# microsoft/fadtk

Measured on NVIDIA H100. Metric: audio_seconds_embedded_per_second, higher is better.
Workload: dtype f16

## Files before the change

fadtk_b200/_native.py:

```python
from __future__ import annotations

import ctypes as C
import os
from pathlib import Path

import numpy as np
import torch

_LIB_PATH = Path(os.environ.get("FADTK_B200_LIB") or Path(__file__).parent / "csrc" / "libfadtk_b200.so")
_lib = None

c_ll = C.c_longlong
c_vp = C.c_void_p


class NativeError(RuntimeError):
    pass


class VggishWeights(C.Structure):
    _fields_ = [("conv1_w_host", c_vp), ("conv1_b_host", c_vp),
                ("conv_w_host", c_vp * 5), ("conv_b_host", c_vp * 5),
                ("fc_w_host", c_vp * 3), ("fc_b_host", c_vp * 3), ("split_mask", C.c_uint32)]


SIGNATURES = {
    "fad_version": (C.c_int, []),
    "fad_last_error": (C.c_char_p, []),
    "fad_create": (C.c_int, [C.c_int, C.c_int, C.POINTER(c_vp)]),
    "fad_destroy": (C.c_int, [c_vp]),
    "fad_vggish_load": (C.c_int, [c_vp, C.POINTER(VggishWeights)]),
    "fad_vggish_num_examples": (c_ll, [c_ll]),
    "fad_vggish_plan": (c_ll, [c_vp, c_ll, c_vp, c_ll, c_vp]),
    "fad_vggish_forward": (C.c_int, [c_vp, c_vp, c_vp, c_ll, c_vp, c_vp]),
    "fad_vggish_logmel": (C.c_int, [c_vp, c_vp, c_vp, c_ll, c_vp, C.c_int, c_vp]),
    "fad_vggish_conv1": (C.c_int, [c_vp, c_vp, c_ll, c_vp, c_vp]),
    "fad_umma_layer": (C.c_int, [c_vp, c_vp, C.c_int, C.c_int, C.c_int, C.c_int, c_vp, c_vp,
                                 C.c_int, C.c_int, C.c_int, C.c_int, C.c_int, c_vp, c_vp, c_vp]),
    "fad_linear": (C.c_int, [c_vp, c_vp, c_ll, C.c_int, c_ll, c_vp, C.c_int, c_vp, C.c_int, C.c_int, c_vp, c_vp,
                             c_vp, C.c_int, C.c_int, C.c_int, c_vp]),
    "fad_clap_load": (C.c_int, [c_vp, c_vp, C.c_int, C.c_int]),
    "fad_clap_plan": (c_ll, [c_vp, c_ll, c_vp, c_vp, c_ll, c_vp]),
    "fad_clap_plan_frames": (c_ll, [c_vp, c_ll, c_vp, c_vp, c_vp, c_ll, c_vp]),
    "fad_clap_forward": (C.c_int, [c_vp, c_vp, c_vp, c_vp, c_vp, c_ll, c_vp, c_ll, c_vp, c_vp]),
    "fad_clap_logmel": (C.c_int, [c_vp, c_vp, c_vp, c_vp, c_vp, c_ll, c_vp, c_vp]),
    "fad_clap_patch_embed": (C.c_int, [c_vp, c_vp, c_ll, c_vp, c_ll, c_vp, c_vp]),
    "fad_clap_block": (C.c_int, [c_vp, C.c_int, c_vp, c_ll, c_vp, c_vp]),
    "fad_clap_merge": (C.c_int, [c_vp, C.c_int, c_vp, c_ll, c_vp, c_vp]),
    "fad_clap_head": (C.c_int, [c_vp, c_vp, c_ll, c_vp, c_vp]),
    "fad_stats_acc_len": (C.c_size_t, [C.c_int]),
    "fad_stats_accumulate": (C.c_int, [c_vp, c_vp, c_ll, C.c_int, c_vp, c_vp, C.c_int, c_vp]),
    "fad_stats_accumulate_gather": (C.c_int, [c_vp, c_vp, c_ll, c_vp, c_ll, C.c_int, c_vp, c_vp, c_vp]),
    "fad_stats_finalize": (C.c_int, [c_vp, c_vp, c_vp, C.c_int, c_vp, c_vp, c_vp]),
    "fad_file_means": (C.c_int, [c_vp, c_vp, c_ll, C.c_int, C.c_int, c_vp, c_vp, c_vp]),
    "fad_stats_accumulate_f64": (C.c_int, [c_vp, c_vp, c_ll, C.c_int, c_vp, c_vp]),
    "fad_stats_finalize_mirrored": (C.c_int, [c_vp, c_vp, c_vp, c_vp, c_vp, C.c_int, C.c_int, c_vp, c_vp, c_vp]),
    "fad_frechet": (C.c_int, [c_vp, c_vp, c_vp, c_vp, c_vp, C.c_int, C.c_int, c_vp, c_vp]),
    "fad_sqrt_psd": (C.c_int, [c_vp, c_vp, C.c_int, C.c_int, c_vp, c_vp, c_vp]),
    "fad_frechet_presqrt": (C.c_int, [c_vp, c_vp, c_vp, c_vp, c_vp, c_vp, C.c_int, C.c_int, c_vp, c_vp]),
    "fad_whisper_load": (C.c_int, [c_vp, c_vp, c_vp, C.c_int, C.c_int]),
    "fad_whisper_forward": (C.c_int, [c_vp, c_vp, c_vp, c_vp, c_ll, c_vp, c_vp]),
    "fad_whisper_logmel": (C.c_int, [c_vp, c_vp, c_vp, c_vp, c_ll, c_vp, c_vp]),
    "fad_whisper_conv": (C.c_int, [c_vp, C.c_int, c_vp, c_vp, c_ll, c_vp, c_vp]),
    "fad_whisper_enc_layer": (C.c_int, [c_vp, C.c_int, c_vp, c_ll, c_vp, c_vp]),
    "fad_whisper_encode": (C.c_int, [c_vp, c_vp, c_vp, c_vp, c_ll, c_vp, c_vp]),
    "fad_whisper_dec_layer": (C.c_int, [c_vp, C.c_int, c_vp, c_vp, c_ll, c_vp, c_vp]),
    "fad_w2v_load": (C.c_int, [c_vp, c_vp, c_vp, C.c_int, C.c_int, C.c_int]),
    "fad_w2v_forward": (C.c_int, [c_vp, c_vp, c_ll, C.c_int, C.c_int, c_vp, c_vp]),
    "fad_w2v_normalize": (C.c_int, [c_vp, c_vp, c_ll, C.c_int, c_vp, c_vp]),
    "fad_w2v_conv": (C.c_int, [c_vp, C.c_int, c_vp, c_ll, C.c_int, c_vp, c_vp]),
    "fad_w2v_posconv": (C.c_int, [c_vp, c_vp, c_ll, C.c_int, c_vp, c_vp]),
    "fad_w2v_layer": (C.c_int, [c_vp, C.c_int, c_vp, c_ll, C.c_int, c_vp, c_vp]),
    "fad_encodec_load": (C.c_int, [c_vp, c_vp, C.c_int, c_ll, C.c_int]),
    "fad_encodec_forward": (C.c_int, [c_vp, c_vp, c_ll, C.c_int, c_vp, c_vp]),
    "fad_encodec_conv": (C.c_int, [c_vp, C.c_int, c_vp, c_ll, C.c_int, C.c_int, C.c_int, c_vp, c_vp]),
    "fad_encodec_lstm": (C.c_int, [c_vp, c_vp, c_ll, C.c_int, c_vp, c_vp]),
    "fad_resample_geometry": (C.c_int, [C.c_int, C.c_int, c_vp, c_vp, c_vp, c_vp]),
    "fad_resample_length": (c_ll, [C.c_int, C.c_int, c_ll]),
    "fad_resample_bank": (C.c_int, [C.c_int, C.c_int, c_vp]),
    "fad_resample": (C.c_int, [c_vp, c_vp, c_vp, C.c_int, c_ll, C.c_int, C.c_int, c_vp, c_vp, c_vp]),
    "fad_frechet_batched": (C.c_int, [c_vp, c_vp, c_vp, c_vp, c_vp, c_vp, c_ll, C.c_int, C.c_int, c_vp, c_vp]),
    "fad_attention": (C.c_int, [c_vp, c_vp, c_ll, C.c_int, C.c_int, c_vp, C.c_int, c_vp]),
    "fad_window_attention": (C.c_int, [c_vp, c_vp, c_ll, C.c_int, C.c_int, c_vp, C.c_int, C.c_int, c_vp, c_vp]),
    "fad_attention_bias": (C.c_int, [c_vp, c_vp, c_ll, C.c_int, C.c_int, c_vp, c_vp, c_vp, c_vp]),
    "fad_wavlm_gate": (C.c_int, [c_vp, c_vp, c_vp, c_vp, c_vp, c_ll, C.c_int, C.c_int, c_vp, c_vp]),
    "fad_wavlm_bias_table": (C.c_int, [C.c_int, C.c_int, c_vp, c_vp]),
    "fad_decoder_self_attention": (C.c_int, [c_vp, c_vp, c_ll, C.c_int, c_vp, c_vp]),
    "fad_cross_attention": (C.c_int, [c_vp, c_vp, c_vp, c_ll, C.c_int, C.c_int, c_vp, c_vp]),
    "fad_layernorm": (C.c_int, [c_vp, c_vp, c_vp, c_vp, c_ll, C.c_int, C.c_int, C.c_int, C.c_int, C.c_int, C.c_int,
                                c_vp, c_vp, c_vp]),
    "fad_bench_dmma_peak": (C.c_int, [c_vp, C.c_int, c_vp]),
    "fad_kad_median_sq": (C.c_int, [c_vp, c_vp, c_ll, C.c_int, c_vp, c_vp]),
    "fad_kad_sums": (C.c_int, [c_vp, c_vp, c_ll, c_ll, C.c_int, c_vp, c_vp, c_vp]),
    "fad_kad_song_sums": (C.c_int, [c_vp, c_vp, c_ll, c_vp, c_ll, C.c_int, c_vp, c_vp, c_vp]),
    "fad_kad_median_sq_sharded": (C.c_int, [c_vp, c_vp, C.c_int, c_vp, c_ll, C.c_int, c_vp, c_vp]),
    "fad_kad_sums_sharded": (C.c_int, [c_vp, c_vp, C.c_int, c_vp, c_ll, c_ll, C.c_int, c_vp, c_vp, c_vp]),
    "fad_kad_song_sums_sharded": (C.c_int, [c_vp, c_vp, C.c_int, c_vp, c_ll, c_vp, c_ll, C.c_int, c_vp, c_vp, c_vp]),
    "fad_kad_shard_plan": (C.c_int, [c_vp, c_ll, C.c_int, c_vp]),
    "fad_knn_radii_sq": (C.c_int, [c_vp, c_vp, c_ll, c_ll, C.c_int, C.c_int, c_vp, c_vp]),
    "fad_prdc_counts": (C.c_int, [c_vp, c_vp, c_ll, c_ll, C.c_int, c_vp, c_vp, c_vp, c_vp]),
    "fad_comm_unique_id": (C.c_int, [c_vp]),
    "fad_comm_init": (C.c_int, [c_vp, c_vp, C.c_int, C.c_int]),
    "fad_comm_destroy": (C.c_int, [c_vp]),
    "fad_stats_allreduce": (C.c_int, [c_vp, c_vp, c_vp, C.c_int, c_vp]),
    "fad_allreduce_sum_f64": (C.c_int, [c_vp, c_vp, c_vp, c_ll, c_vp]),
    "fad_launch_count": (c_ll, [c_vp]),
    "fad_profile_enable": (C.c_int, [c_vp, C.c_int]),
    "fad_profile_collect": (C.c_int, [c_vp, c_vp, c_vp, C.c_int]),
}

PROF_CATEGORIES = 20
PROF_NAMES = {0: "logmel", 1: "conv1", 2: "conv2", 3: "conv3_1", 4: "conv3_2", 5: "conv4_1", 6: "conv4_2",
              7: "fc1", 8: "fc2", 9: "fc3", 10: "stats", 11: "stats_reduce", 12: "frechet",
              13: "clap_front", 14: "clap_gemm", 15: "clap_attn", 16: "clap_other"}


def library_path() -> Path:
    return _LIB_PATH


def lib():
    global _lib
    if _lib is None:
        if not _LIB_PATH.exists():
            raise NativeError(
                f"{_LIB_PATH} is missing - run `python -c 'import __graft_entry__ as g; g.build()'`. "
                "fadtk_b200 has no CPU fallback.")
        _lib = C.CDLL(str(_LIB_PATH))
        for name, (res, args) in SIGNATURES.items():
            fn = getattr(_lib, name)
            fn.restype = res
            fn.argtypes = args
    return _lib


def _check(rc: int):
    if rc != 0:
        raise NativeError(lib().fad_last_error().decode())


def _stream() -> int:
    return torch.cuda.current_stream().cuda_stream


def _ptr(t) -> int:
    return 0 if t is None else t.data_ptr()


class Engine:

    def __init__(self, device: int | None = None, max_examples: int = 2048):
        if not torch.cuda.is_available():
            raise NativeError("no CUDA device visible: fadtk_b200 has no CPU fallback")
        self.device = torch.cuda.current_device() if device is None else int(device)
        self.max_examples = int(max_examples)
        h = c_vp()
        _check(lib().fad_create(self.device, self.max_examples, C.byref(h)))
        self._h = h
        self._keep = []
        self.has_comm = False
        self.owners = {}

    def close(self):
        if getattr(self, "_h", None):
            lib().fad_destroy(self._h)
            self._h = None

    def __del__(self):
        try:
            self.close()
        except Exception:
            pass

    @property
    def torch_device(self):
        return torch.device("cuda", self.device)

    @property
    def launches(self) -> int:
        return int(lib().fad_launch_count(self._h))

    @staticmethod
    def comm_unique_id() -> bytes:
        buf = C.create_string_buffer(128)
        _check(lib().fad_comm_unique_id(buf))
        return buf.raw

    def comm_init(self, unique_id: bytes, rank: int, world: int):
        assert len(unique_id) == 128
        _check(lib().fad_comm_init(self._h, C.create_string_buffer(unique_id, 128), int(rank), int(world)))
        self.has_comm = True

    def allreduce_sum_(self, buf: torch.Tensor) -> torch.Tensor:
        assert buf.dtype == torch.float64 and buf.is_cuda and buf.is_contiguous()
        _check(lib().fad_allreduce_sum_f64(self._h, None, buf.data_ptr(), buf.numel(), _stream()))
        return buf

    def attention(self, qkv: torch.Tensor, n_clips: int, legacy: bool = False) -> torch.Tensor:
        assert qkv.dtype == torch.float16 and qkv.is_cuda and qkv.is_contiguous() and qkv.shape[0] % n_clips == 0
        S, d = qkv.shape[0] // n_clips, qkv.shape[1] // 3
        out = torch.empty((qkv.shape[0], d), dtype=torch.float16, device=qkv.device)
        _check(lib().fad_attention(self._h, qkv.data_ptr(), n_clips, S, d, out.data_ptr(), int(legacy), _stream()))
        return out

    def window_attention(self, qkv, n_windows: int, C: int, heads: int, relbias, res: int, shift: int, out):
        _check(lib().fad_window_attention(self._h, _ptr(qkv), int(n_windows), int(C), int(heads), _ptr(relbias),
                                          int(res), int(shift), _ptr(out), _stream()))
        return out

    def attention_bias(self, qkv, n_clips: int, S: int, d: int, relb, gate, out):
        _check(lib().fad_attention_bias(self._h, _ptr(qkv), int(n_clips), int(S), int(d), _ptr(relb), _ptr(gate),
                                        _ptr(out), _stream()))
        return out

    def wavlm_gate(self, x, w, b, c, rows: int, heads: int, d: int, out):
        _check(lib().fad_wavlm_gate(self._h, _ptr(x), _ptr(w), _ptr(b), _ptr(c), int(rows), int(heads), int(d),
                                    _ptr(out), _stream()))
        return out

    @staticmethod
    def wavlm_bias_table(rel_embed: np.ndarray, S: int) -> np.ndarray:
        emb = np.ascontiguousarray(rel_embed, dtype=np.float32)
        out = np.empty((emb.shape[1], max(2 * int(S) - 1, 0)), dtype=np.float32)
        _check(lib().fad_wavlm_bias_table(emb.shape[1], int(S), emb.ctypes.data, out.ctypes.data))
        return out

    def decoder_self_attention(self, qkv, n_clips: int, d: int, out):
        _check(lib().fad_decoder_self_attention(self._h, _ptr(qkv), int(n_clips), int(d), _ptr(out), _stream()))
        return out

    def cross_attention(self, q, kv, n_clips: int, S: int, d: int, out):
        _check(lib().fad_cross_attention(self._h, _ptr(q), _ptr(kv), int(n_clips), int(S), int(d), _ptr(out), _stream()))
        return out

    def layernorm(self, x, gamma, beta, rows: int, C: int, ld_out: int, out16, out32=None, *, res: int = 0,
                  shift: int = 0, mode: int = 0, gelu: bool = False):
        _check(lib().fad_layernorm(self._h, _ptr(x), _ptr(gamma), _ptr(beta), int(rows), int(C), int(ld_out), int(res),
                                   int(shift), int(mode), int(gelu), _ptr(out16), _ptr(out32), _stream()))
        return out16

    def dmma_peak_tflops(self, iters: int = 0) -> float:
        out = C.c_double(0.0)
        _check(lib().fad_bench_dmma_peak(self._h, int(iters), C.byref(out)))
        return float(out.value)

    def profile(self, on: bool):
        _check(lib().fad_profile_enable(self._h, int(on)))

    def profile_collect(self, reset: bool = True) -> dict:
        ms = (C.c_double * PROF_CATEGORIES)()
        cnt = (c_ll * PROF_CATEGORIES)()
        _check(lib().fad_profile_collect(self._h, ms, cnt, int(reset)))
        return {PROF_NAMES[i]: (ms[i], int(cnt[i])) for i in PROF_NAMES if cnt[i]}

    def vggish_load(self, packed: dict):
        self.owners.pop("vggish", None)
        w = VggishWeights()
        keep = {k: v.contiguous() for k, v in packed.items() if hasattr(v, "contiguous")}
        w.conv1_w_host = keep["conv1.w"].data_ptr()
        w.conv1_b_host = keep["conv1.b"].data_ptr()
        for i in range(5):
            w.conv_w_host[i] = keep[f"conv{i + 2}.w"].data_ptr()
            w.conv_b_host[i] = keep[f"conv{i + 2}.b"].data_ptr()
        for i in range(3):
            w.fc_w_host[i] = keep[f"fc{i + 1}.w"].data_ptr()
            w.fc_b_host[i] = keep[f"fc{i + 1}.b"].data_ptr()
        w.split_mask = int(packed.get("split_mask", 0))
        _check(lib().fad_vggish_load(self._h, C.byref(w)))

    @staticmethod
    def vggish_plan(clip_offsets: np.ndarray):
        off = np.ascontiguousarray(clip_offsets, dtype=np.int64)
        n_clips = off.shape[0] - 1
        rows = np.empty(n_clips, dtype=np.int64)
        n = lib().fad_vggish_plan(off.ctypes.data, n_clips, None, 0, rows.ctypes.data)
        ex = np.empty(n, dtype=np.int64)
        lib().fad_vggish_plan(off.ctypes.data, n_clips, ex.ctypes.data, n, None)
        return ex, rows

    def vggish_forward(self, pcm: torch.Tensor, ex_start: torch.Tensor, out: torch.Tensor | None = None):
        assert pcm.dtype == torch.int16 and pcm.is_cuda and pcm.is_contiguous()
        assert ex_start.dtype == torch.int64 and ex_start.is_cuda
        n = ex_start.shape[0]
        if out is None:
            out = torch.empty((n, 128), dtype=torch.float16, device=pcm.device)
# ... 432 lines not shown
```

fadtk_b200/csrc/fadtk_b200.cu:

```cuda
#include "../../include/fadtk_b200.h"

#include <cuda.h>
#include <cuda_runtime.h>
#include <cuda_fp16.h>
#include <cxxabi.h>
#include <algorithm>
#include <cmath>
#include <cstdio>
#include <cstdlib>
#include <cstring>
#include <memory>
#include <set>
#include <string>
#include <type_traits>
#include <utility>
#include <vector>

#include "conv_gemm.cuh"
#include "frontend.cuh"
#include "stats.cuh"
#include "frechet.cuh"
#include "clap.cuh"
#include "resample.cuh"
#include "whisper.cuh"
// ... 429 lines not shown
    if (!h) return fail("null handle");
    h->prof_on = on != 0;
    return 0;
}

int fad_profile_collect(fad_handle* h, double* ms_out, long long* count_out, int reset) {
    if (!h) return fail("null handle");
    CK(cudaSetDevice(h->device));
    CK(cudaDeviceSynchronize());
    for (const auto& sp : h->spans) {
        float ms = 0.f;
        if (cudaEventElapsedTime(&ms, h->ev_pool[sp.e0], h->ev_pool[sp.e1]) == cudaSuccess) {
            h->prof_ms[sp.cat] += ms; h->prof_count[sp.cat]++;
        }
    }
    h->spans.clear(); h->ev_used = 0;
    for (int i = 0; i < FAD_PROF_CATEGORIES; ++i) {
        if (ms_out) ms_out[i] = h->prof_ms[i];
        if (count_out) count_out[i] = h->prof_count[i];
        if (reset) { h->prof_ms[i] = 0.0; h->prof_count[i] = 0; }
    }
    return 0;
}
const char* fad_last_error(void) { return g_err.c_str(); }

int fad_create(int device, int max_examples, fad_handle** out) {
    if (!out) return fail("null out pointer");
    int count = 0;
    if (cudaGetDeviceCount(&count) != cudaSuccess || count == 0)
        return fail("no CUDA device: fadtk_b200 has no CPU fallback");
    if (device < 0 || device >= count) return fail("bad device index");
    CK(cudaSetDevice(device));
    cudaDeviceProp prop;
    CK(cudaGetDeviceProperties(&prop, device));
    if (prop.major != 9) return fail("fadtk_b200 kernels are built for sm_90a (Hopper H100) only");
    std::unique_ptr<fad_handle> h(new fad_handle());
    h->device = device;
    h->num_sms = prop.multiProcessorCount;
    h->max_examples = max_examples > 0 ? max_examples : 2048;

    std::vector<double> tw, hann, melw; std::vector<int> ms, mc;
    build_frontend_tables(tw, hann, melw, ms, mc);
    if (upload(h->mem, &h->d_twiddle, tw.data(), tw.size() * 8) || upload(h->mem, &h->d_hann, hann.data(), hann.size() * 8) ||
        upload(h->mem, &h->d_melw, melw.data(), melw.size() * 8) || upload(h->mem, &h->d_mel_start, ms.data(), ms.size() * 4) ||
        upload(h->mem, &h->d_mel_count, mc.data(), mc.size() * 4)) return 1;
    const auto smem = [](const void* kernel, size_t bytes) {
        return cudaFuncSetAttribute(kernel, cudaFuncAttributeMaxDynamicSharedMemorySize, (int)bytes);
    };
    CK(smem((const void*)fad::logmel_kernel<double>, fad::logmel_smem_bytes<double>()));
    CK(smem((const void*)fad::logmel_kernel<float>, fad::logmel_smem_bytes<float>()));
    CK(smem((const void*)fad::clap_logmel_kernel, fad::clap_logmel_smem_bytes()));
    CK(smem((const void*)fad::attention_wgmma_kernel, fad::kAtSmem));
    CK(smem((const void*)fad::clap_window_attention_kernel<24>, fad::att_smem_bytes(24, fad::kAttWarps, fad::kAttStages)));
    CK(smem((const void*)fad::clap_window_attention_kernel<32>, fad::att_smem_bytes(32, fad::kAttWarps, fad::kAttStages)));
    CK(smem((const void*)fad::kad_tile_kernel<0>, fad::kKadSmemBytes));
    CK(smem((const void*)fad::kad_tile_kernel<1>, fad::kKadSmemBytes));
    CK(smem((const void*)fad::kad_tile_kernel<2>, fad::kKadSmemBytes));
    CK(smem((const void*)fad::prdc_tile_kernel<0>, fad::kPrdcSmemBytes));
    CK(smem((const void*)fad::prdc_tile_kernel<1>, fad::kPrdcSmemBytes));
    if (setup_gemm<0>(h.get()) || setup_gemm<1>(h.get())) return 1;
    *out = h.release();
    return 0;
}

int fad_destroy(fad_handle* h) {
    if (!h) return 0;
    cudaSetDevice(h->device);
    fad_comm_destroy(h);
    delete h;
    return 0;
}

long long fad_launch_count(fad_handle* h) { return h ? h->launches : 0; }

int fad_vggish_load(fad_handle* h, const fad_vggish_weights* w) {
    if (!h || !w) return fail("null argument");
    const void* src[18] = {w->conv1_w_host, w->conv1_b_host,
                           w->conv_w_host[0], w->conv_w_host[1], w->conv_w_host[2], w->conv_w_host[3], w->conv_w_host[4],
                           w->fc_w_host[0], w->fc_w_host[1], w->fc_w_host[2],
                           w->conv_b_host[0], w->conv_b_host[1], w->conv_b_host[2], w->conv_b_host[3], w->conv_b_host[4],
                           w->fc_b_host[0], w->fc_b_host[1], w->fc_b_host[2]};
    if (check_tensors("fad_vggish_load", src, 18)) return 1;
    const void* const* wsrc = src + 2;
    const void* const* bsrc = src + 10;
    CK(cudaSetDevice(h->device));
    h->vgg.reset();
    auto vs = std::make_unique<VggState>();
    auto& m = vs->mem;
    if (upload(m, &vs->conv1_w, src[0], 64 * 9 * 4) || upload(m, &vs->conv1_b, src[1], 64 * 4)) return 1;
    for (int i = 0; i < 8; ++i) {
        const VggLayer& L = kVgg[i];
        const size_t mul = ((w->split_mask >> i) & 1) ? 2 : 1;
        if (upload(m, &vs->w[i], wsrc[i], mul * L.Cout * L.taps * L.Cin * 2) || upload(m, &vs->b[i], bsrc[i], (size_t)L.Cout * 4))
            return 1;
    }
    for (int i = 0; i < 8; ++i)
        if (((w->split_mask >> i) & 1) &&
            note_split_weights(h, vs->w[i], kVgg[i].Cout / 128, (long long)kVgg[i].taps * kVgg[i].Cin, 0)) return 1;
    const size_t B = (size_t)h->max_examples;
    if (alloc(m, &vs->logmel, B * 96 * 64 * 4)) return 1;
    for (int i = 0; i < 8; ++i)
        if (alloc(m, &vs->act[i], B * kActElems[i] * 2)) return 1;
    for (int i = 0; i < 8; ++i) {
        const VggLayer& L = kVgg[i];
        if (make_geom(vs->geom[i], L.H, L.W, L.Cin, L.Cout, L.taps, L.relu, L.pool, (w->split_mask >> i) & 1)) return 1;
        if (encode_layer_maps(vs->geom[i], vs->act[i], (long long)B, vs->w[i], &vs->map_x[i], &vs->map_w[i])) return 1;
    }
    h->vgg = std::move(vs);
    return 0;
}

long long fad_vggish_num_examples(long long n_samples) {
    if (n_samples < fad::kWin) return 0;
    const long long t = 1 + (n_samples - fad::kWin) / fad::kHop;
    if (t < fad::kExFrames) return 0;
    return 1 + (t - fad::kExFrames) / fad::kExFrames;
}

long long fad_vggish_plan(const long long* clip_offsets_host, long long n_clips,
                          long long* ex_start_host, long long capacity, long long* rows_per_clip_host) {
    long long n = 0;
    for (long long c = 0; c < n_clips; ++c) {
        const long long len = clip_offsets_host[c + 1] - clip_offsets_host[c];
        const long long k = fad_vggish_num_examples(len);
        if (rows_per_clip_host) rows_per_clip_host[c] = k;
        for (long long e = 0; e < k; ++e, ++n)
            if (ex_start_host && n < capacity)
                ex_start_host[n] = clip_offsets_host[c] + e * (long long)(fad::kExFrames * fad::kHop);
    }
    return n;
}

static int launch_logmel(fad_handle* h, const int16_t* pcm, const long long* ex_start, long long n,
                         float* out, int use_double, cudaStream_t st) {
    fad::FrontendTables tab{h->d_twiddle, h->d_hann, h->d_melw, h->d_mel_start, h->d_mel_count};
    const long long frames = n * fad::kExFrames;
    long long blocks = (frames + fad::kFeWarps - 1) / fad::kFeWarps;
    const long long cap = (long long)h->num_sms * 8;
    if (blocks > cap) blocks = cap;
    if (use_double)
        return launch(h, fad::logmel_kernel<double>, (int)blocks, fad::kFeWarps * 32, fad::logmel_smem_bytes<double>(), st,
                      pcm, ex_start, (int)n, tab, out);
    return launch(h, fad::logmel_kernel<float>, (int)blocks, fad::kFeWarps * 32, fad::logmel_smem_bytes<float>(), st,
                  pcm, ex_start, (int)n, tab, out);
}

int fad_vggish_logmel(fad_handle* h, const int16_t* pcm, const long long* ex_start,
                      long long n_examples, float* logmel_out, int use_double, void* stream) {
    if (!h) return fail("null handle");
    CK(cudaSetDevice(h->device));
    return launch_logmel(h, pcm, ex_start, n_examples, logmel_out, use_double, (cudaStream_t)stream);
}

int fad_vggish_forward(fad_handle* h, const int16_t* pcm, const long long* ex_start,
                       long long n_examples, void* emb_out_f16, void* stream) {
    if (!h) return fail("null handle");
    if (!h->vgg) return fail("fad_vggish_load has not been called");
    CK(cudaSetDevice(h->device));
    const VggState& vs = *h->vgg;
    cudaStream_t st = (cudaStream_t)stream;
    static const int fe_double = []() { const char* e = getenv("FADTK_FRONTEND_FP64"); return (e && e[0] == '1') ? 1 : 0; }();
    for (long long base = 0; base < n_examples; base += h->max_examples) {
        const int nb = (int)((n_examples - base) < h->max_examples ? (n_examples - base) : h->max_examples);
        size_t ev = prof_begin(h, st);
        if (launch_logmel(h, pcm, ex_start + base, nb, vs.logmel, fe_double, st)) return 1;
        prof_end(h, FAD_PROF_LOGMEL, ev, st);
        ev = prof_begin(h, st);
        if (launch(h, fad::conv1_kernel, dim3(6, nb), 256, 0, st, vs.logmel, vs.conv1_w, vs.conv1_b, vs.act[0])) return 1;
        prof_end(h, FAD_PROF_CONV1, ev, st);
        for (int i = 0; i < 8; ++i) {
            void* out = (i == 7) ? (void*)((__half*)emb_out_f16 + (size_t)base * 128) : (void*)vs.act[i + 1];
            ev = prof_begin(h, st);
            if (run_layer(h, vs.geom[i], vs.map_x[i], vs.map_w[i], vs.w[i], nb, vs.b[i], out, nullptr, st)) return 1;
            prof_end(h, FAD_PROF_LAYER0 + i, ev, st);
        }
    }
    return 0;
}

int fad_vggish_conv1(fad_handle* h, const float* logmel, long long n_examples, void* out_f16, void* stream) {
    if (!h) return fail("null handle");
    if (!h->vgg) return fail("fad_vggish_load has not been called");
    if (n_examples <= 0) return 0;
    CK(cudaSetDevice(h->device));
    return launch(h, fad::conv1_kernel, dim3(6, (unsigned)n_examples), 256, 0, (cudaStream_t)stream,
                  logmel, h->vgg->conv1_w, h->vgg->conv1_b, reinterpret_cast<__half*>(out_f16));
}

int fad_umma_layer(fad_handle* h, const void* x_f16, int NB, int H, int W, int Cin,
                   const void* w_f16, const float* bias, int Cout, int taps, int relu, int pool,
                   int split_w, void* out_f16, float* out_f32_or_null, void* stream) {
    if (!h) return fail("null handle");
    if (split_w != 0 && split_w != 1) return fail("fad_umma_layer: split_w must be 0 (fp16 weights) or 1 (fp16 hi/lo pair)");
    CK(cudaSetDevice(h->device));
    LayerGeom g;
    if (make_geom(g, H, W, Cin, Cout, taps, relu, pool, split_w)) return 1;
    if (pool && out_f32_or_null) return fail("fp32 copy is only available for un-pooled layers");
    if (g.split_w == 1 && note_split_weights(h, w_f16, Cout / 128, (long long)taps * Cin, (cudaStream_t)stream)) return 1;
    CUtensorMap mx, mw;
    if (encode_layer_maps(g, x_f16, NB, w_f16, &mx, &mw)) return 1;
    return run_layer(h, g, mx, mw, w_f16, NB, bias, out_f16, out_f32_or_null, (cudaStream_t)stream);
}

size_t fad_stats_acc_len(int d) { return 1 + 2 * (size_t)d + (size_t)d * d; }

int fad_stats_accumulate(fad_handle* h, const void* emb_f16, long long n_rows, int d,
                         const void* shift_f16, double* acc, int tensor_core, void* stream) {
    if (!h) return fail("null handle");
    if (tensor_core != 0 && tensor_core != 2) return fail("fad_stats_accumulate: tensor_core must be 0 (DMMA) or 2 (CUDA-core fp64)");
    if (n_rows <= 0) return 0;
    CK(cudaSetDevice(h->device));
    cudaStream_t st = (cudaStream_t)stream;
    const __half* E = reinterpret_cast<const __half*>(emb_f16);
    const __half* shift = reinterpret_cast<const __half*>(shift_f16);
    if (tensor_core == 0) return launch_stats_dmma(h, E, n_rows, d, shift, acc, st);
    if (d % 64 != 0) return fail("d must be a multiple of 64");
    dim3 grid((unsigned)((n_rows + fad::kSimtRows - 1) / fad::kSimtRows), d / 64, d / 64);
    return launch(h, fad::stats_simt_kernel, grid, 256, 0, st, E, n_rows, d, shift, acc);
}

int fad_file_means(fad_handle* h, const void* emb_f16, long long n_files, int rows_per_file, int d,
                   double* m64_out, double* m16_out, void* stream) {
    if (!h) return fail("null handle");
    if (n_files <= 0) return 0;
    if (rows_per_file <= 0 || d <= 0) return fail("bad shape");
    CK(cudaSetDevice(h->device));
    long long blocks = (n_files * d + 255) / 256;
    if (blocks > (long long)h->num_sms * 16) blocks = (long long)h->num_sms * 16;
    return launch(h, fad::file_means_kernel, (unsigned)blocks, 256, 0, (cudaStream_t)stream,
                  reinterpret_cast<const __half*>(emb_f16), n_files, rows_per_file, d, m64_out, m16_out);
}

int fad_stats_accumulate_f64(fad_handle* h, const double* rows, long long n_rows, int d, double* acc, void* stream) {
    if (!h) return fail("null handle");
    if (n_rows <= 0) return 0;
    CK(cudaSetDevice(h->device));
    return launch_stats_dmma(h, rows, n_rows, d, nullptr, acc, (cudaStream_t)stream);
}

int fad_stats_finalize_mirrored(fad_handle* h, const double* acc, const double* acc_means64, const double* acc_means16,
                                const void* shift_f16, int rows_per_file, int d, double* mu_out, double* cov_out, void* stream) {
    if (!h) return fail("null handle");
    CK(cudaSetDevice(h->device));
    static const int keep = [] { const char* e = getenv("FADTK_SINGLE_FRAME_FILES"); return (e && std::string(e) == "keep") ? 1 : 0; }();
    const size_t total = (size_t)d * d;
    unsigned blocks = (unsigned)((total + 255) / 256);
    if (blocks > (unsigned)h->num_sms * 8) blocks = h->num_sms * 8;
    return launch(h, fad::stats_finalize_mirrored_kernel, blocks, 256, 0, (cudaStream_t)stream,
                  acc, acc_means64, acc_means16, reinterpret_cast<const __half*>(shift_f16), rows_per_file, d, keep, mu_out, cov_out);
}

int fad_stats_accumulate_gather(fad_handle* h, const void* emb_f16, long long n_src_rows,
                                const long long* idx, long long n_idx, int d,
                                const void* shift_f16, double* acc, void* stream) {
    if (!h) return fail("null handle");
    (void)n_src_rows;
    if (n_idx <= 0) return 0;
    if (d % 8 != 0) return fail("d must be a multiple of 8");
    CK(cudaSetDevice(h->device));
    if (h->gather_buf.grow((size_t)n_idx * d * 2)) return 1;
    __half* rows = h->gather_buf.get<__half>();
    const long long vecs = n_idx * (d / 8);
    long long blocks = (vecs + 255) / 256;
    if (blocks > (long long)h->num_sms * 16) blocks = (long long)h->num_sms * 16;
    if (launch(h, fad::gather_rows_kernel, (unsigned)blocks, 256, 0, (cudaStream_t)stream,
               reinterpret_cast<const __half*>(emb_f16), idx, n_idx, d, rows)) return 1;
    return launch_stats_dmma(h, rows, n_idx, d, reinterpret_cast<const __half*>(shift_f16), acc, (cudaStream_t)stream);
}

int fad_stats_finalize(fad_handle* h, const double* acc, const void* shift_f16, int d,
                       double* mu_out, double* cov_out, void* stream) {
    if (!h) return fail("null handle");
    CK(cudaSetDevice(h->device));
    const size_t total = (size_t)d * d;
    unsigned blocks = (unsigned)((total + 255) / 256);
    if (blocks > (unsigned)h->num_sms * 8) blocks = h->num_sms * 8;
    return launch(h, fad::stats_finalize_kernel, blocks, 256, 0, (cudaStream_t)stream,
                  acc, reinterpret_cast<const __half*>(shift_f16), d, mu_out, cov_out);
}

extern "C" int fad_attention(fad_handle* h, const void* qkv_f16, long long n_clips, int S, int d, void* out_f16, int legacy, void* stream) {
    if (!h || !qkv_f16 || !out_f16) return fail("null argument");
    if (d % 64 != 0 || S <= 0 || n_clips <= 0) return fail("bad shape");
    CK(cudaSetDevice(h->device));
    cudaStream_t st = (cudaStream_t)stream;
    if (!legacy) return launch_attention_wgmma(h, reinterpret_cast<const __half*>(qkv_f16), n_clips, S, d, d / 64, reinterpret_cast<__half*>(out_f16), st);
    return launch(h, fad::whisper_flash_attention_kernel, dim3((S + 63) / 64, d / 64, (unsigned)n_clips), 128, 0, st,
                  reinterpret_cast<const __half*>(qkv_f16), S, d, reinterpret_cast<__half*>(out_f16), nullptr, nullptr);
}


#include <dlfcn.h>
namespace {
struct NcclId { char bytes[128]; };
struct NcclApi {
    int (*GetUniqueId)(NcclId*) = nullptr;
    int (*CommInitRank)(void**, int, NcclId, int) = nullptr;
    int (*AllReduce)(const void*, void*, size_t, int, int, void*, cudaStream_t) = nullptr;
    int (*CommDestroy)(void*) = nullptr;
    int (*CommCount)(void*, int*) = nullptr;
    int (*CommUserRank)(void*, int*) = nullptr;
    const char* (*GetErrorString)(int) = nullptr;
    bool ok = false;
    std::string why;
};
NcclApi& nccl_api() {
    static NcclApi api = [] {
        NcclApi a;
        const char* env = getenv("FADTK_NCCL_LIB");
        const char* names[] = {env, "libnccl.so.2", "libnccl.so"};
        void* lib = nullptr;
        for (const char* n : names) {
            if (!n || !*n) continue;
            lib = dlopen(n, RTLD_NOW | RTLD_GLOBAL);
            if (lib) break;
        }
        if (!lib) { a.why = "libnccl.so.2 not found (set FADTK_NCCL_LIB)"; return a; }
        a.GetUniqueId = reinterpret_cast<decltype(a.GetUniqueId)>(dlsym(lib, "ncclGetUniqueId"));
        a.CommInitRank = reinterpret_cast<decltype(a.CommInitRank)>(dlsym(lib, "ncclCommInitRank"));
        a.AllReduce = reinterpret_cast<decltype(a.AllReduce)>(dlsym(lib, "ncclAllReduce"));
        a.CommDestroy = reinterpret_cast<decltype(a.CommDestroy)>(dlsym(lib, "ncclCommDestroy"));
        a.CommCount = reinterpret_cast<decltype(a.CommCount)>(dlsym(lib, "ncclCommCount"));
        a.CommUserRank = reinterpret_cast<decltype(a.CommUserRank)>(dlsym(lib, "ncclCommUserRank"));
        a.GetErrorString = reinterpret_cast<decltype(a.GetErrorString)>(dlsym(lib, "ncclGetErrorString"));
        a.ok = a.GetUniqueId && a.CommInitRank && a.AllReduce && a.CommDestroy && a.CommCount && a.CommUserRank &&
               a.GetErrorString;
        if (!a.ok) a.why = "NCCL library lacks an expected symbol";
        return a;
    }();
    return api;
}
int nccl_fail(const char* what, int rc) {
    return fail(std::string(what) + ": " + (nccl_api().GetErrorString ? nccl_api().GetErrorString(rc) : "NCCL error"));
}
}

extern "C" {
int fad_comm_unique_id(void* id_out_host) {
    if (!id_out_host) return fail("null argument");
// ... 696 lines not shown
```

fadtk_b200/csrc/frontend.cuh:

```cuda
#pragma once
#include <cuda_fp16.h>
#include <stdint.h>

namespace fad {

constexpr int kWin = 400, kHop = 160, kFft = 512, kBins = 257, kMel = 64, kExFrames = 96;
constexpr int kMelMaxTaps = 24;
constexpr int kFeWarps = 8;

struct FrontendTables {
    const double* twiddle;
    const double* hann;
    const double* mel_w;
    const int* mel_start;
    const int* mel_count;
};

template <typename T> struct Cx { T re, im; };

template <typename T>
__host__ __device__ constexpr size_t logmel_smem_bytes() {
    return sizeof(T) * (size_t)(kFeWarps * (2 * 256 + 260) + 2 * 256 + kWin + kMel * kMelMaxTaps)
         + sizeof(int) * 2 * kMel;
}

template <typename T> __device__ __forceinline__ Cx<T> cmul(Cx<T> a, Cx<T> b) {
    return {a.re * b.re - a.im * b.im, a.re * b.im + a.im * b.re};
}
template <typename T> __device__ __forceinline__ Cx<T> cadd(Cx<T> a, Cx<T> b) { return {a.re + b.re, a.im + b.im}; }
template <typename T> __device__ __forceinline__ Cx<T> csub(Cx<T> a, Cx<T> b) { return {a.re - b.re, a.im - b.im}; }
template <typename T> __device__ __forceinline__ Cx<T> mul_neg_i(Cx<T> a) { return {a.im, -a.re}; }

template <typename T> __device__ __forceinline__ void fft8(Cx<T> (&a)[8]) {
    const T c = (T)0.70710678118654752440;
    Cx<T> b0 = cadd(a[0], a[4]), b4 = csub(a[0], a[4]);
    Cx<T> b1 = cadd(a[1], a[5]), t1 = csub(a[1], a[5]);
    Cx<T> b2 = cadd(a[2], a[6]), b6 = mul_neg_i(csub(a[2], a[6]));
    Cx<T> b3 = cadd(a[3], a[7]), t3 = csub(a[3], a[7]);
    Cx<T> b5 = {c * (t1.re + t1.im), c * (t1.im - t1.re)};
    Cx<T> b7 = {c * (t3.im - t3.re), -c * (t3.re + t3.im)};
    Cx<T> q0 = cadd(b0, b2), q1 = cadd(b1, b3), q2 = csub(b0, b2), q3 = mul_neg_i(csub(b1, b3));
    a[0] = cadd(q0, q1); a[4] = csub(q0, q1); a[2] = cadd(q2, q3); a[6] = csub(q2, q3);
    Cx<T> r0 = cadd(b4, b6), r1 = cadd(b5, b7), r2 = csub(b4, b6), r3 = mul_neg_i(csub(b5, b7));
    a[1] = cadd(r0, r1); a[5] = csub(r0, r1); a[3] = cadd(r2, r3); a[7] = csub(r2, r3);
}

__device__ __forceinline__ float shfl_xor_t(float v, int m) { return __shfl_xor_sync(0xffffffffu, v, m); }
__device__ __forceinline__ double shfl_xor_t(double v, int m) { return __shfl_xor_sync(0xffffffffu, v, m); }

template <typename T>
__global__ void __launch_bounds__(kFeWarps * 32)
logmel_kernel(const int16_t* __restrict__ pcm, const long long* __restrict__ ex_start,
              int n_examples, FrontendTables tab, float* __restrict__ out)
{
    extern __shared__ __align__(16) unsigned char fe_smem[];
    T* sm = reinterpret_cast<T*>(fe_smem);
    Cx<T>* tw = reinterpret_cast<Cx<T>*>(sm);
    T* hann = sm + 512;
    T* melw = hann + kWin;
    T* wbuf = melw + kMel * kMelMaxTaps;
    int* mstart = reinterpret_cast<int*>(wbuf + kFeWarps * (512 + 260));
    int* mcount = mstart + kMel;

    for (int i = threadIdx.x; i < 256; i += blockDim.x) {
        tw[i].re = (T)tab.twiddle[2 * i]; tw[i].im = (T)tab.twiddle[2 * i + 1];
    }
    for (int i = threadIdx.x; i < kWin; i += blockDim.x) hann[i] = (T)tab.hann[i];
    for (int i = threadIdx.x; i < kMel * kMelMaxTaps; i += blockDim.x) melw[i] = (T)tab.mel_w[i];
    for (int i = threadIdx.x; i < kMel; i += blockDim.x) { mstart[i] = tab.mel_start[i]; mcount[i] = tab.mel_count[i]; }
    __syncthreads();

    const int warp = threadIdx.x >> 5, lane = threadIdx.x & 31;
    Cx<T>* z = reinterpret_cast<Cx<T>*>(wbuf + warp * (512 + 260));
    T* mag = wbuf + warp * (512 + 260) + 512;

    T hw[7][2];
#pragma unroll
    for (int n1 = 0; n1 < 7; ++n1) {
        const int n = 32 * n1 + lane;
        hw[n1][0] = n < kWin / 2 ? hann[2 * n] * (T)(1.0 / 32768.0) : (T)0;
        hw[n1][1] = n < kWin / 2 ? hann[2 * n + 1] * (T)(1.0 / 32768.0) : (T)0;
    }
    Cx<T> tw1[8];
#pragma unroll
    for (int k1 = 0; k1 < 8; ++k1) {
        const int m = 2 * lane * k1;
        const Cx<T> w = tw[m & 255];
        tw1[k1] = (m & 256) ? Cx<T>{-w.re, -w.im} : w;
    }
    Cx<T> tw2[5];
#pragma unroll
    for (int s = 0; s < 5; ++s) {
        const int h = 16 >> s;
        tw2[s] = tw[(lane & (h - 1)) * (256 / h)];
    }
    const int rev = __brev((unsigned)lane) >> 27;

    const long long total = (long long)n_examples * kExFrames;
    for (long long g = (long long)blockIdx.x * kFeWarps + warp; g < total;
         g += (long long)gridDim.x * kFeWarps) {
        const int e = (int)(g / kExFrames), f = (int)(g % kExFrames);
        const int16_t* src = pcm + ex_start[e] + (long long)f * kHop;

        Cx<T> a[8];
#pragma unroll
        for (int n1 = 0; n1 < 7; ++n1) {
            const int n = 32 * n1 + lane;
            if (n < kWin / 2) {
                a[n1].re = (T)src[2 * n] * hw[n1][0];
                a[n1].im = (T)src[2 * n + 1] * hw[n1][1];
            } else { a[n1].re = 0; a[n1].im = 0; }
        }
        a[7].re = 0; a[7].im = 0;
        fft8(a);
#pragma unroll
        for (int k1 = 1; k1 < 8; ++k1) a[k1] = cmul(a[k1], tw1[k1]);
#pragma unroll
        for (int s = 0; s < 5; ++s) {
            const int h = 16 >> s;
            const bool upper = (lane & h) != 0;
#pragma unroll
            for (int r = 0; r < 8; ++r) {
                Cx<T> p = {shfl_xor_t(a[r].re, h), shfl_xor_t(a[r].im, h)};
                a[r] = upper ? cmul(csub(p, a[r]), tw2[s]) : cadd(a[r], p);
            }
        }
#pragma unroll
        for (int k1 = 0; k1 < 8; ++k1) z[k1 + 8 * rev] = a[k1];
        __syncwarp();
        for (int k = lane; k <= 128; k += 32) {
            const Cx<T> x = z[k], y = z[(256 - k) & 255];
            const T er = (T)0.5 * (x.re + y.re), ei = (T)0.5 * (x.im - y.im);
            const T orr = (T)0.5 * (x.im + y.im), oi = (T)-0.5 * (x.re - y.re);
            const Cx<T> w = tw[k & 255];
            const T pr = orr * w.re - oi * w.im, pi = orr * w.im + oi * w.re;
            const T xr = er + pr, xi = ei + pi, yr = er - pr, yi = ei - pi;
            mag[k] = sqrt(xr * xr + xi * xi);
            mag[256 - k] = sqrt(yr * yr + yi * yi);
        }
        __syncwarp();
        float* dst = out + g * kMel;
#pragma unroll
        for (int hsel = 0; hsel < 2; ++hsel) {
            const int b = hsel ? 63 - lane : lane;
            const int st = mstart[b], cnt = mcount[b];
            T acc = 0;
            for (int i = 0; i < cnt; ++i) acc += mag[st + i] * melw[b * kMelMaxTaps + i];
            dst[b] = (float)log(acc + (T)0.01);
        }
        __syncwarp();
    }
}

__device__ __forceinline__ void mma_m16n8k16(float (&c)[4], uint32_t a0, uint32_t a1, uint32_t a2, uint32_t a3,
                                             uint32_t b0, uint32_t b1) {
    asm volatile("mma.sync.aligned.m16n8k16.row.col.f32.f16.f16.f32 {%0,%1,%2,%3}, {%4,%5,%6,%7}, {%8,%9}, {%0,%1,%2,%3};"
                 : "+f"(c[0]), "+f"(c[1]), "+f"(c[2]), "+f"(c[3])
                 : "r"(a0), "r"(a1), "r"(a2), "r"(a3), "r"(b0), "r"(b1));
}

__global__ void __launch_bounds__(256)
conv1_kernel(const float* __restrict__ logmel , const float* __restrict__ w ,
             const float* __restrict__ bias, __half* __restrict__ out )
{
    __shared__ float tile[18][68];
    const int e = blockIdx.y, strip = blockIdx.x;
    const int row0 = strip * 16 - 1;
    const float* src = logmel + (size_t)e * 96 * 64;
    for (int i = threadIdx.x; i < 18 * 66; i += 256) {
        const int r = i / 66, c = i % 66;
        const int gr = row0 + r, gc = c - 1;
        tile[r][c] = (gr >= 0 && gr < 96 && gc >= 0 && gc < 64) ? src[gr * 64 + gc] : 0.0f;
    }
    const int lane = threadIdx.x & 31, warp = threadIdx.x >> 5;
    float w0[9], w1[9];
#pragma unroll
    for (int i = 0; i < 9; ++i) { w0[i] = w[(2 * lane) * 9 + i]; w1[i] = w[(2 * lane + 1) * 9 + i]; }
    const float b0 = bias[2 * lane], b1 = bias[2 * lane + 1];
    __syncthreads();

    const int py = warp;
#pragma unroll 2
    for (int px = 0; px < 32; ++px) {
        float patch[4][4];
#pragma unroll
        for (int r = 0; r < 4; ++r)
#pragma unroll
            for (int c = 0; c < 4; ++c) patch[r][c] = tile[2 * py + r][2 * px + c];
        float m0 = -3.0e38f, m1 = -3.0e38f;
#pragma unroll
        for (int dy = 0; dy < 2; ++dy)
#pragma unroll
            for (int dx = 0; dx < 2; ++dx) {
                float a0 = 0.f, a1 = 0.f;
#pragma unroll
                for (int kh = 0; kh < 3; ++kh)
#pragma unroll
                    for (int kw = 0; kw < 3; ++kw) {
                        const float x = patch[dy + kh][dx + kw];
                        a0 = fmaf(w0[kh * 3 + kw], x, a0);
                        a1 = fmaf(w1[kh * 3 + kw], x, a1);
                    }
                m0 = fmaxf(m0, a0); m1 = fmaxf(m1, a1);
            }
        m0 = fmaxf(m0 + b0, 0.f); m1 = fmaxf(m1 + b1, 0.f);
        const size_t pix = ((size_t)e * 48 + strip * 8 + py) * 32 + px;
        *reinterpret_cast<__half2*>(out + pix * 64 + 2 * lane) = __floats2half2_rn(m0, m1);
    }
}

}
```

Measured before the change: 180,800.

## Restructure conv1 kernel for register reuse, vector loads and taller strips

```diff
diff --git a/fadtk_b200/_native.py b/fadtk_b200/_native.py
--- a/fadtk_b200/_native.py
+++ b/fadtk_b200/_native.py
@@ -119,18 +119,24 @@
     return _LIB_PATH
 
 
+def load(path) -> C.CDLL:
+    path = Path(path)
+    if not path.exists():
+        raise NativeError(
+            f"{path} is missing - run `python -c 'import __graft_entry__ as g; g.build()'`. "
+            "fadtk_b200 has no CPU fallback.")
+    so = C.CDLL(str(path))
+    for name, (res, args) in SIGNATURES.items():
+        fn = getattr(so, name)
+        fn.restype = res
+        fn.argtypes = args
+    return so
+
+
 def lib():
     global _lib
     if _lib is None:
-        if not _LIB_PATH.exists():
-            raise NativeError(
-                f"{_LIB_PATH} is missing - run `python -c 'import __graft_entry__ as g; g.build()'`. "
-                "fadtk_b200 has no CPU fallback.")
-        _lib = C.CDLL(str(_LIB_PATH))
-        for name, (res, args) in SIGNATURES.items():
-            fn = getattr(_lib, name)
-            fn.restype = res
-            fn.argtypes = args
+        _lib = load(_LIB_PATH)
     return _lib
 
 
diff --git a/fadtk_b200/csrc/fadtk_b200.cu b/fadtk_b200/csrc/fadtk_b200.cu
--- a/fadtk_b200/csrc/fadtk_b200.cu
+++ b/fadtk_b200/csrc/fadtk_b200.cu
@@ -605,6 +605,12 @@
     return launch_logmel(h, pcm, ex_start, n_examples, logmel_out, use_double, (cudaStream_t)stream);
 }
 
+static int launch_conv1(fad_handle* h, const float* logmel, long long n, const float* w, const float* b, __half* out,
+                        cudaStream_t st) {
+    if (reinterpret_cast<uintptr_t>(logmel) % 16) return fail("conv1: log-mel input must be 16-byte aligned");
+    return launch(h, fad::conv1_kernel, dim3(fad::kExFrames / (2 * fad::kC1Rows), (unsigned)n), 256, 0, st, logmel, w, b, out);
+}
+
 int fad_vggish_forward(fad_handle* h, const int16_t* pcm, const long long* ex_start,
                        long long n_examples, void* emb_out_f16, void* stream) {
     if (!h) return fail("null handle");
@@ -619,7 +625,7 @@
         if (launch_logmel(h, pcm, ex_start + base, nb, vs.logmel, fe_double, st)) return 1;
         prof_end(h, FAD_PROF_LOGMEL, ev, st);
         ev = prof_begin(h, st);
-        if (launch(h, fad::conv1_kernel, dim3(6, nb), 256, 0, st, vs.logmel, vs.conv1_w, vs.conv1_b, vs.act[0])) return 1;
+        if (launch_conv1(h, vs.logmel, nb, vs.conv1_w, vs.conv1_b, vs.act[0], st)) return 1;
         prof_end(h, FAD_PROF_CONV1, ev, st);
         for (int i = 0; i < 8; ++i) {
             void* out = (i == 7) ? (void*)((__half*)emb_out_f16 + (size_t)base * 128) : (void*)vs.act[i + 1];
@@ -636,8 +642,8 @@
     if (!h->vgg) return fail("fad_vggish_load has not been called");
     if (n_examples <= 0) return 0;
     CK(cudaSetDevice(h->device));
-    return launch(h, fad::conv1_kernel, dim3(6, (unsigned)n_examples), 256, 0, (cudaStream_t)stream,
-                  logmel, h->vgg->conv1_w, h->vgg->conv1_b, reinterpret_cast<__half*>(out_f16));
+    return launch_conv1(h, logmel, n_examples, h->vgg->conv1_w, h->vgg->conv1_b, reinterpret_cast<__half*>(out_f16),
+                        (cudaStream_t)stream);
 }
 
 int fad_umma_layer(fad_handle* h, const void* x_f16, int NB, int H, int W, int Cin,
diff --git a/fadtk_b200/csrc/frontend.cuh b/fadtk_b200/csrc/frontend.cuh
--- a/fadtk_b200/csrc/frontend.cuh
+++ b/fadtk_b200/csrc/frontend.cuh
@@ -159,54 +159,70 @@
                  : "r"(a0), "r"(a1), "r"(a2), "r"(a3), "r"(b0), "r"(b1));
 }
 
+constexpr int kC1Rows = 16;
 __global__ void __launch_bounds__(256)
 conv1_kernel(const float* __restrict__ logmel , const float* __restrict__ w ,
              const float* __restrict__ bias, __half* __restrict__ out )
 {
-    __shared__ float tile[18][68];
+    __shared__ __align__(16) float tile[2 * kC1Rows + 2][68];
     const int e = blockIdx.y, strip = blockIdx.x;
-    const int row0 = strip * 16 - 1;
-    const float* src = logmel + (size_t)e * 96 * 64;
-    for (int i = threadIdx.x; i < 18 * 66; i += 256) {
-        const int r = i / 66, c = i % 66;
-        const int gr = row0 + r, gc = c - 1;
-        tile[r][c] = (gr >= 0 && gr < 96 && gc >= 0 && gc < 64) ? src[gr * 64 + gc] : 0.0f;
-    }
-    const int lane = threadIdx.x & 31, warp = threadIdx.x >> 5;
-    float w0[9], w1[9];
-#pragma unroll
-    for (int i = 0; i < 9; ++i) { w0[i] = w[(2 * lane) * 9 + i]; w1[i] = w[(2 * lane + 1) * 9 + i]; }
-    const float b0 = bias[2 * lane], b1 = bias[2 * lane + 1];
+    const int row0 = strip * 2 * kC1Rows - 1;
+    const float4* src = reinterpret_cast<const float4*>(logmel + (size_t)e * 96 * 64);
+    for (int i = threadIdx.x; i < (2 * kC1Rows + 2) * 16; i += 256) {
+        const int r = i >> 4, c4 = i & 15, gr = row0 + r;
+        const float4 v = (gr >= 0 && gr < 96) ? src[gr * 16 + c4] : make_float4(0.f, 0.f, 0.f, 0.f);
+        float* d = &tile[r][4 * c4 + 1];
+        d[0] = v.x; d[1] = v.y; d[2] = v.z; d[3] = v.w;
+    }
+    if (threadIdx.x < 2 * (2 * kC1Rows + 2)) tile[threadIdx.x >> 1][(threadIdx.x & 1) ? 65 : 0] = 0.f;
+    const int lane = threadIdx.x & 31, c0 = 4 * (lane & 15);
+    const int py = 2 * (threadIdx.x >> 5) + (lane >> 4);
+    float wk[4][9], bk[4];
+#pragma unroll
+    for (int c = 0; c < 4; ++c) {
+#pragma unroll
+        for (int i = 0; i < 9; ++i) wk[c][i] = w[(c0 + c) * 9 + i];
+        bk[c] = bias[c0 + c];
+    }
     __syncthreads();
 
-    const int py = warp;
+    const float* trow = &tile[2 * py][0];
+    __half* dst = out + (((size_t)e * 48 + strip * kC1Rows + py) * 32) * 64 + c0;
+    float x[4][4];
+#pragma unroll
+    for (int r = 0; r < 4; ++r) {
+        const float2 v = *reinterpret_cast<const float2*>(trow + r * 68);
+        x[r][0] = v.x; x[r][1] = v.y;
+    }
 #pragma unroll 2
     for (int px = 0; px < 32; ++px) {
-        float patch[4][4];
-#pragma unroll
-        for (int r = 0; r < 4; ++r)
-#pragma unroll
-            for (int c = 0; c < 4; ++c) patch[r][c] = tile[2 * py + r][2 * px + c];
-        float m0 = -3.0e38f, m1 = -3.0e38f;
+#pragma unroll
+        for (int r = 0; r < 4; ++r) {
+            const float2 v = *reinterpret_cast<const float2*>(trow + r * 68 + 2 * px + 2);
+            x[r][2] = v.x; x[r][3] = v.y;
+        }
+        float m[4] = {-3.0e38f, -3.0e38f, -3.0e38f, -3.0e38f};
 #pragma unroll
         for (int dy = 0; dy < 2; ++dy)
 #pragma unroll
             for (int dx = 0; dx < 2; ++dx) {
-                float a0 = 0.f, a1 = 0.f;
+                float acc[4] = {0.f, 0.f, 0.f, 0.f};
 #pragma unroll
                 for (int kh = 0; kh < 3; ++kh)
 #pragma unroll
-                    for (int kw = 0; kw < 3; ++kw) {
-                        const float x = patch[dy + kh][dx + kw];
-                        a0 = fmaf(w0[kh * 3 + kw], x, a0);
-                        a1 = fmaf(w1[kh * 3 + kw], x, a1);
-                    }
-                m0 = fmaxf(m0, a0); m1 = fmaxf(m1, a1);
+                    for (int kw = 0; kw < 3; ++kw)
+#pragma unroll
+                        for (int c = 0; c < 4; ++c) acc[c] = fmaf(wk[c][kh * 3 + kw], x[dy + kh][dx + kw], acc[c]);
+#pragma unroll
+                for (int c = 0; c < 4; ++c) m[c] = fmaxf(m[c], acc[c]);
             }
-        m0 = fmaxf(m0 + b0, 0.f); m1 = fmaxf(m1 + b1, 0.f);
-        const size_t pix = ((size_t)e * 48 + strip * 8 + py) * 32 + px;
-        *reinterpret_cast<__half2*>(out + pix * 64 + 2 * lane) = __floats2half2_rn(m0, m1);
-    }
-}
-
-}
+        const __half2 lo = __floats2half2_rn(fmaxf(m[0] + bk[0], 0.f), fmaxf(m[1] + bk[1], 0.f));
+        const __half2 hi = __floats2half2_rn(fmaxf(m[2] + bk[2], 0.f), fmaxf(m[3] + bk[3], 0.f));
+        *reinterpret_cast<uint2*>(dst + px * 64) = make_uint2(*reinterpret_cast<const uint32_t*>(&lo),
+                                                              *reinterpret_cast<const uint32_t*>(&hi));
+#pragma unroll
+        for (int r = 0; r < 4; ++r) { x[r][0] = x[r][2]; x[r][1] = x[r][3]; }
+    }
+}
+
+}
```

Result: no change. 181,200, median of 6 (+0.2%).
